# shaohua-pan/RobustCap

Hardware: AMD Instinct MI355X
Metric: body-frames/sec (sig_mp fwd + FK) at batch 256 (higher is better)
Workload: dtype f32; 1 GPU; synthetic 60 fps, 6 IMU + 33 keypoints, batch 256 x 1448 frames per GPU (256 bodies in total, weak scaling), confidence schedule 'mixed', seeded random weights (63.4 M params); batch_per_gpu=256, bodies_total=256, frames=1448, conf=mixed, parallelism=dp1 (sequence sharding)

## Files before the change

### include/robustcap_hip.h

```cpp
#ifndef ROBUSTCAP_HIP_H
#define ROBUSTCAP_HIP_H

#include <stdint.h>

#ifdef __cplusplus
extern "C" {
#endif

typedef struct rc_ctx rc_ctx;

typedef enum {
    RC_OK = 0,
    RC_ERR_INVALID = -1,
    RC_ERR_HIP = -2,
    RC_ERR_STATE = -3,
    RC_ERR_UNKNOWN_KEY = -4
} rc_status;

typedef struct {
    double conf_lo, conf_hi;
    float contact_threshold;
    float distance_threshold;
    float height_threshold;
    double tran_filter_num;
// ... 16 lines not shown
int rc_get_params(const rc_ctx* ctx, rc_params* out);
int rc_set_params(rc_ctx* ctx, const rc_params* p);

int rc_load_weight(rc_ctx* ctx, const char* key, const float* host, int64_t numel);
int rc_finalize_weights(rc_ctx* ctx);

int rc_set_body(rc_ctx* ctx, const int32_t* parent, const float* J, const float* w33, const float* v33);

int rc_set_gravity(rc_ctx* ctx, const float* gravity_host);

int rc_reset(rc_ctx* ctx, const uint8_t* row_mask, void* stream);

int rc_step(rc_ctx* ctx, const float* j2dc, const float* accc, const float* oric, const float* first_tran,
            uint32_t flags, float* pose_out, float* tran_out, void* stream);

int rc_sequence(rc_ctx* ctx, int32_t T, const float* j2dc, int64_t rs_j2d, const float* accc, int64_t rs_acc,
                const float* oric, int64_t rs_ori, const float* first_tran, uint32_t flags, float* pose_out,
                int64_t rs_pose, float* tran_out, int64_t rs_tran, void* stream);

int rc_sequence_rows(rc_ctx* ctx, int32_t T, const int32_t* len_host, const float* j2dc, int64_t rs_j2d, const float* accc,
                     int64_t rs_acc, const float* oric, int64_t rs_ori, const float* first_tran, uint32_t flags, float* pose_out,
                     int64_t rs_pose, float* tran_out, int64_t rs_tran, void* stream);
int rc_get_sequence_row_frames(rc_ctx* ctx, int64_t* body_frames);

int rc_set_gemm_mode(rc_ctx* ctx, int32_t mode);
int rc_get_gemm_mode(const rc_ctx* ctx);
int rc_default_gemm_mode(int32_t total_rows);
int rc_initial_gemm_mode(int32_t total_rows);

int rc_set_sequence_mode(rc_ctx* ctx, int32_t mode, int32_t min_frames);
int rc_get_sequence_stats(rc_ctx* ctx, int64_t* wave_frames, int64_t* stepped_frames, int64_t* ticks);
int rc_get_launch_stats(rc_ctx* ctx, int64_t* lds_launches, int64_t* other_wide_launches);
int rc_get_launch_stats_w32(rc_ctx* ctx, int64_t* w32_launches);
int rc_set_resident(rc_ctx* ctx, int32_t enable, int32_t workgroups);
int rc_get_resident_stats(rc_ctx* ctx, int64_t* segments, int64_t* aborts);
int rc_plan_sequence(const int8_t* codes, int32_t B, int32_t T, const int32_t* pend, uint32_t flags, int32_t use_vision_updater,
                     uint8_t* mode_out);
int rc_plan_wave(const int8_t* codes, int32_t B, int32_t T, int32_t t0, const int32_t* first_reach, const int32_t* pend,
                 int32_t use_imu_updater, int32_t use_vision_updater, int32_t* frame_at, int64_t frame_at_cap,
                 int32_t* n_ticks, int32_t* n_prep, int32_t* counts, double* est_us);
int rc_plan_wave_rows(const int8_t* codes, int32_t B, int32_t T, int32_t t0, const int32_t* len, const int32_t* first_reach,
                      const int32_t* pend, int32_t use_imu_updater, int32_t use_vision_updater, int32_t* frame_at, int64_t frame_at_cap,
                      int32_t* n_ticks, int32_t* n_prep, int32_t* counts, double* est_us);

int rc_live_begin(rc_ctx* ctx);
int rc_live_step(rc_ctx* ctx, const float* j2dc_host, const float* accc_host, const float* oric_host,
                 const float* first_tran_host, uint32_t flags, float* pose_host, float* tran_host);
int rc_live_end(rc_ctx* ctx);
int rc_get_live_stats(rc_ctx* ctx, int64_t* lean_frames, int64_t* full_frames);
int rc_get_live_prestep(rc_ctx* ctx, int64_t* presteps, int32_t* available);
int rc_get_live_replayed(rc_ctx* ctx, int64_t* frames);
int rc_get_live_spin(rc_ctx* ctx, int64_t* taken, int64_t* lost);
int rc_get_live_profile(rc_ctx* ctx, double* avg_us4);
int rc_get_live_last_profile(rc_ctx* ctx, double* us6);
int rc_get_live_backend(rc_ctx* ctx, int32_t* lean_captured, int32_t* aql, char* note, int32_t note_len);

int rc_r6d_to_rotmat(const float* r6d, float* R, int64_t n, void* stream);
int rc_axis_angle_to_rotmat(const float* aa, float* R, int64_t n, void* stream);
int rc_rotmat_to_axis_angle(const float* R, float* aa, int64_t n, void* stream);
int rc_rotmat_to_r6d(const float* R, float* r6d, int64_t n, void* stream);
int rc_angle_between(const float* R1, const float* R2, float* out, int64_t n, void* stream);
int rc_lerp(const float* a, const float* b, double t, float* out, int64_t n, void* stream);
int rc_normalize_rows(const float* x, float* out, float* norm, int64_t rows, int32_t width, void* stream);
int rc_bbox_normalise(const float* kp, float* out, int64_t n, void* stream);
int rc_conf_mean(const float* j2dc, int64_t n, double lo, double hi, float* mean, int8_t* code, void* stream);
int rc_shape_body(rc_ctx* ctx, const float* v_template, const float* shapedirs, const float* J_regressor, const float* beta,
// ... 142 lines not shown
```

### robustcap_amd/_lib.py

```python
import ctypes as C
import os

_HERE = os.path.dirname(os.path.abspath(__file__))
LIB_PATH = os.environ.get("RC_LIB_PATH") or os.path.join(_HERE, "csrc", "librobustcap_hip.so")
HEADER_PATH = os.path.join(os.path.dirname(_HERE), "include", "robustcap_hip.h")

RC_FLAG_FIRST_FRAME = 1


class RcParams(C.Structure):
    _fields_ = [("conf_lo", C.c_double), ("conf_hi", C.c_double),
                ("contact_threshold", C.c_float), ("distance_threshold", C.c_float),
                ("height_threshold", C.c_float), ("tran_filter_num", C.c_double),
                ("use_flat_floor", C.c_int32), ("use_vision_updater", C.c_int32),
                ("use_imu_updater", C.c_int32), ("live", C.c_int32),
                ("update_vision_freq", C.c_int32), ("use_reproj_opt", C.c_int32), ("smooth", C.c_float),
                ("reserved", C.c_int32)]


class RcSmplifyInfo(C.Structure):
    _fields_ = [("status", C.c_int32), ("n_iter", C.c_int32), ("n_eval", C.c_int32), ("reserved", C.c_int32),
                ("first_loss", C.c_double), ("final_loss", C.c_double), ("host_ms", C.c_double), ("device_ms", C.c_double)]


OBJECTIVE_FN = C.CFUNCTYPE(C.c_double, C.c_void_p, C.POINTER(C.c_double), C.POINTER(C.c_double), C.c_int64)


class RobustcapLibraryError(RuntimeError):
    pass


_P, _I32, _I64, _U32, _F = C.c_void_p, C.c_int32, C.c_int64, C.c_uint32, C.c_float
SIGNATURES = {
    "rc_create": (_I32, [_I32, _I32, C.POINTER(_P)]),
    "rc_destroy": (_I32, [_P]),
    "rc_last_error": (C.c_char_p, [_P]),
    "rc_default_params": (_I32, [_I32, C.POINTER(RcParams)]),
    "rc_get_params": (_I32, [_P, C.POINTER(RcParams)]),
    "rc_set_params": (_I32, [_P, C.POINTER(RcParams)]),
    "rc_load_weight": (_I32, [_P, C.c_char_p, _P, _I64]),
    "rc_finalize_weights": (_I32, [_P]),
    "rc_set_body": (_I32, [_P, _P, _P, _P, _P]),
    "rc_set_gravity": (_I32, [_P, _P]),
    "rc_reset": (_I32, [_P, _P, _P]),
    "rc_step": (_I32, [_P, _P, _P, _P, _P, _U32, _P, _P, _P]),
    "rc_sequence": (_I32, [_P, _I32, _P, _I64, _P, _I64, _P, _I64, _P, _U32, _P, _I64, _P, _I64, _P]),
    "rc_sequence_rows": (_I32, [_P, _I32, _P, _P, _I64, _P, _I64, _P, _I64, _P, _U32, _P, _I64, _P, _I64, _P]),
    "rc_get_sequence_row_frames": (_I32, [_P, C.POINTER(_I64)]),
    "rc_set_gemm_mode": (_I32, [_P, _I32]),
    "rc_get_gemm_mode": (_I32, [_P]),
    "rc_default_gemm_mode": (_I32, [_I32]),
    "rc_initial_gemm_mode": (_I32, [_I32]),
    "rc_set_sequence_mode": (_I32, [_P, _I32, _I32]),
    "rc_get_sequence_stats": (_I32, [_P, C.POINTER(_I64), C.POINTER(_I64), C.POINTER(_I64)]),
    "rc_get_launch_stats": (_I32, [_P, C.POINTER(_I64), C.POINTER(_I64)]),
    "rc_get_launch_stats_w32": (_I32, [_P, C.POINTER(_I64)]),
    "rc_set_resident": (_I32, [_P, _I32, _I32]),
    "rc_get_resident_stats": (_I32, [_P, C.POINTER(_I64), C.POINTER(_I64)]),
    "rc_plan_sequence": (_I32, [_P, _I32, _I32, _P, _U32, _I32, _P]),
    "rc_plan_wave": (_I32, [_P, _I32, _I32, _I32, _P, _P, _I32, _I32, _P, _I64, C.POINTER(_I32), C.POINTER(_I32), _P, _P]),
    "rc_plan_wave_rows": (_I32, [_P, _I32, _I32, _I32, _P, _P, _P, _I32, _I32, _P, _I64, C.POINTER(_I32), C.POINTER(_I32), _P, _P]),
    "rc_live_begin": (_I32, [_P]),
    "rc_live_step": (_I32, [_P, _P, _P, _P, _P, _U32, _P, _P]),
    "rc_live_end": (_I32, [_P]),
    "rc_get_live_stats": (_I32, [_P, _P, _P]),
    "rc_get_live_prestep": (_I32, [_P, _P, _P]),
    "rc_get_live_replayed": (_I32, [_P, _P]),
    "rc_get_live_spin": (_I32, [_P, _P, _P]),
    "rc_get_live_profile": (_I32, [_P, _P]),
    "rc_get_live_last_profile": (_I32, [_P, _P]),
    "rc_get_live_backend": (_I32, [_P, _P, _P, _P, _I32]),
    "rc_get_fusion_state": (_I32, [_P, _P, _P]),
    "rc_r6d_to_rotmat": (_I32, [_P, _P, _I64, _P]),
    "rc_axis_angle_to_rotmat": (_I32, [_P, _P, _I64, _P]),
    "rc_rotmat_to_axis_angle": (_I32, [_P, _P, _I64, _P]),
    "rc_rotmat_to_r6d": (_I32, [_P, _P, _I64, _P]),
    "rc_angle_between": (_I32, [_P, _P, _P, _I64, _P]),
    "rc_lerp": (_I32, [_P, _P, C.c_double, _P, _I64, _P]),
    "rc_normalize_rows": (_I32, [_P, _P, _P, _I64, _I32, _P]),
    "rc_bbox_normalise": (_I32, [_P, _P, _I64, _P]),
    "rc_conf_mean": (_I32, [_P, _I64, C.c_double, C.c_double, _P, _P, _P]),
    "rc_shape_body": (_I32, [_P, _P, _P, _P, _P, _I32, _P, _P]),
    "rc_fk_r": (_I32, [_P, _P, _P, _I64, _P]),
    "rc_bone_to_joint": (_I32, [_P, _P, _P, _I64, _P]),
    "rc_joint_to_bone": (_I32, [_P, _P, _P, _I64, _P]),
    "rc_zero_pose": (_I32, [_P, _P, _P, _P]),
    "rc_ik_r": (_I32, [_P, _P, _P, _I64, _P]),
    "rc_fk_bone": (_I32, [_P, _P, _P, _I64, _P]),
    "rc_body_fk": (_I32, [_P, _P, _P, _P, _P, _P, _I64, _P]),
# ... 101 lines not shown
```

### robustcap_amd/csrc/rc_api.cpp

```cpp
#include "../../include/robustcap_hip.h"
#include "rc_ctx.h"

#include <algorithm>
#include <cmath>
#include <cstdio>
#include <cstdlib>
#include <cstring>
#include <map>
#include <string>
#include <thread>
#include <vector>

static thread_local std::string g_create_error;

int fail(rc_ctx* ctx, int code, const std::string& msg) {
    if (ctx) ctx->err = msg; else g_create_error = msg;
    return code;
}

namespace {

const int kInit[3][2] = {{69, 512}, {512, 1024}, {1024, 2048}};

template <typename Body>
// ... 988 lines not shown
        if (ids[i] < 0 || ids[i] > 32) return fail(ctx, RC_ERR_INVALID, "rc_set_ignored_landmarks: id outside 0..32");
        m |= 1ull << ids[i];
    }
    ctx->ign_mask = m;
    return RC_OK;
}
int rc_reproj_residual(rc_ctx* ctx, const float* pose, const float* tran, const float* kp, const float* K, float sigma, float* loss,
                       int64_t T, void* stream) {
    if (!ctx || !ctx->have_body) return ctx ? fail(ctx, RC_ERR_STATE, "rc_reproj_residual: body not set") : RC_ERR_INVALID;
    if (T == 0) return RC_OK;
    if (T < 0 || !pose || !tran || !kp || !K || !loss) return fail(ctx, RC_ERR_INVALID, "rc_reproj_residual: null buffer");
    rc_launch_residual(ctx->body, pose, tran, kp, K, sigma, ctx->ign_mask, loss, T, (hipStream_t)stream);
    HIP_TRY(ctx, hipGetLastError());
    return RC_OK;
}

int rc_lstm_step(rc_ctx* ctx, const char* net, const float* x, const uint8_t* row_mask, float* y, void* stream) {
    if (!ctx || !net || !x || !y) return RC_ERR_INVALID;
    if (!ctx->have_weights) return fail(ctx, RC_ERR_STATE, "rc_lstm_step: weights not finalized");
    const int ni = net_index(net);
    if (ni < 0) return fail(ctx, RC_ERR_INVALID, std::string("rc_lstm_step: unknown net ") + net);
    hipStream_t st = (hipStream_t)stream;
    const NetDev& n = ctx->net[ni];
    if (int rc = flush_pending(ctx, st)) return rc;
    rc_launch_pack_rows(x, n.in, n.in, ctx->xtmp, 256, ctx->B, st);
    Stage s{ni, row_mask ? 255 : 0, ctx->xtmp, 256, Out{y, n.out, 0, false}};
    for (int phase = 0; phase < 4; ++phase) {
        GemmProblem p = phase == 0 ? lin1_problem(ctx, s) : (phase == 3 ? lin2_problem(ctx, s) : lstm_problem(ctx, s, phase - 1));
        if (int rc = launch_problems(ctx, {p}, row_mask, st)) return rc;
    }
    return mark_eager(ctx, st);
}

namespace {
bool camera_constants(const float* K, const float* Tcw, CamConst* cam, float* g_out) {
    for (int q = 0; q < 9; ++q) if (!std::isfinite(K[q])) return false;
    for (int q = 0; q < 12; ++q) if (!std::isfinite(Tcw[q])) return false;
    const double a = K[0], b = K[1], c = K[2], d = K[3], e = K[4], f = K[5], g = K[6], h = K[7], i = K[8];
    const double det = a * (e * i - f * h) - b * (d * i - f * g) + c * (d * h - e * g);
    if (det == 0.0) return false;
    const double inv[9] = {(e * i - f * h) / det, (c * h - b * i) / det, (b * f - c * e) / det,
                           (f * g - d * i) / det, (a * i - c * g) / det, (c * d - a * f) / det,
                           (d * h - e * g) / det, (b * g - a * h) / det, (a * e - b * d) / det};
    for (int q = 0; q < 9; ++q) if (!std::isfinite((float)inv[q])) return false;
    for (int q = 0; q < 9; ++q) cam->Kinv[q] = (float)inv[q];
    for (int r = 0; r < 3; ++r)
        for (int q = 0; q < 3; ++q) cam->R[3 * r + q] = Tcw[4 * r + q];
    for (int r = 0; r < 3; ++r) g_out[r] = -cam->R[3 * r + 1];
    return true;
}
}

int rc_camera_inputs(const float* kp, const float* acc, const float* ori, const float* K, const float* Tcw, float* j2dc,
                     float* accc, float* oric, float* g_out, int64_t n, void* stream) {
    if (!K || !Tcw || !g_out || n < 0) return RC_ERR_INVALID;
    if (n > 0 && (!kp || !acc || !ori || !j2dc || !accc || !oric)) return RC_ERR_INVALID;
    CamConst cam;
    if (!camera_constants(K, Tcw, &cam, g_out)) return RC_ERR_INVALID;
    if (n == 0) return RC_OK;
    rc_launch_camera_inputs(kp, acc, ori, cam, j2dc, accc, oric, n, (hipStream_t)stream);
    return hipGetLastError() == hipSuccess ? RC_OK : RC_ERR_HIP;
}

int rc_camera_inputs_rows(const float* kp_norm, const float* imu_acc_w, const float* imu_ori_w, const int32_t* seq_of_row,
                          const int32_t* len, const float* K_host, const float* Tcw_host, float image_w, float image_h,
                          int32_t n_rows, int32_t Tmax, float* j2dc, float* accc, float* oric, float* gravity_out_host,
// ... 66 lines not shown
```

### robustcap_amd/csrc/rc_ctx.h

```cpp
#pragma once
#include "../../include/robustcap_hip.h"
#include "rc_internal.h"

#include <map>
#include <string>
#include <type_traits>
#include <utility>
#include <vector>

struct NetSpec { const char* name; int in, H, out; };
const NetSpec kNets[6] = {{"rnn2", 72, 512, 69},  {"rnn3", 141, 512, 3},   {"rnn4", 171, 1280, 69},
                          {"rnn6", 240, 1024, 3}, {"rnn7", 141, 512, 144}, {"rnn8", 141, 512, 2}};
enum { N2 = 0, N3 = 1, N4 = 2, N6 = 3, N7 = 4, N8 = 5 };

inline int round_up(int x, int m) { return (x + m - 1) / m * m; }

struct Dense {
    float* W = nullptr; float* b = nullptr;
    void* Ws = nullptr;
    float* Wrm = nullptr;
    int K = 0, N = 0, Kp = 0, Np = 0;
    int mr = 2, nc = 4;
};
struct NetDev {
// ... 70 lines not shown
int tune_env(const char* name, int dflt);
int check_ready(rc_ctx* ctx);
rc_params_dev dev_params(const rc_params& p);
int step_impl(rc_ctx* ctx, const FrameIO& io, uint32_t flags, hipStream_t st, bool with_tr = true, bool skip_prep = false,
              const FrameIO* next_io = nullptr, int n_live = -1);
template <typename T>
int dev_alloc(rc_ctx* ctx, T** p, size_t count, bool zero = true) {
    DevBuf<char> q;
    HIP_TRY(ctx, rc_alloc(q, count * sizeof(T)));
    if (zero) HIP_TRY(ctx, hipMemset(q.get(), 0, count * sizeof(T)));
    *p = reinterpret_cast<T*>(q.get());
    if (!ctx->alloc_weights) ctx->alloc_bytes.emplace_back(q.get(), count * sizeof(T));
    (ctx->alloc_weights ? ctx->weight_allocs : ctx->allocs).push_back(std::move(q));
    return RC_OK;
}
int gemm_create(rc_ctx* ctx);
struct Out { float* p; int ld; int col0; bool packed; };
struct Stage {
    int net; int flag_bit; const float* x; int ldx; Out y;
    const unsigned char* flags = nullptr;
    const float* x_alt = nullptr;
    int sel_bit = 0;
    int out_bit = 0;
    int rows_hint = -1;
};
GemmSeg seg(const float* base, int ld, int K, int mode = RC_PAR_NONE, long long stride = 0);
GemmProblem dense_problem(const rc_ctx* ctx, const Dense& d, GemmSeg a, Out out, bool relu, int flag_bit, const unsigned char* flags, int* steps,
                          bool open_step);
GemmProblem lin1_problem(const rc_ctx* c, const Stage& s);
GemmProblem lstm_problem(const rc_ctx* c, const Stage& s, int layer);
GemmProblem lin2_problem(const rc_ctx* c, const Stage& s);
bool tile_env(const char* name, int* mr, int* nc);
void pick_tile(int H, int rows, int* mr, int* nc);
bool gemm_split(const rc_ctx* c);
int gemm_mode(const rc_ctx* c);
void gemm_planes2_released(rc_ctx* ctx);
int gemm_planes2_ensure(rc_ctx* ctx);
void gemm_planes2_refresh(rc_ctx* ctx, int net, hipStream_t st);
bool lds_context(const rc_ctx* c);
bool lds_problem(const rc_ctx* c, int rows);
struct LdsRegion { float* slab; int* tickets; size_t tiles; };
int lds_region(rc_ctx* ctx, size_t r, LdsRegion* out);
int build_lds_problems(rc_ctx* ctx, const std::vector<GemmProblem>& ps, const unsigned char* flags_override, float* slab, int* tickets,
                       LdsProblem* out, int max_p, int* items, size_t* tiles_out, bool resident_order = false);
int launch_problems(rc_ctx* ctx, std::vector<GemmProblem> ps, const unsigned char* flags_override, hipStream_t st, bool fp32 = false,
                    hipEvent_t stop = nullptr, bool* launched = nullptr);
enum LaunchKind { LAUNCH_SHARED, LAUNCH_WIDE, LAUNCH_SMALL, LAUNCH_RESIDENT };
int timed_launch_impl(rc_ctx* ctx, hipStream_t st, LaunchKind kind, void (*issue)(void*), void* arg);
template <class F> int timed_launch(rc_ctx* ctx, hipStream_t st, LaunchKind kind, F&& issue) {
    return timed_launch_impl(ctx, st, kind, [](void* f) { (*static_cast<std::remove_reference_t<F>*>(f))(); }, &issue);
}
bool resident_launch_fits_timing(const rc_ctx* c);
void count_resident_launch(rc_ctx* ctx);
struct LiveLaunchScope { rc_ctx* ctx; explicit LiveLaunchScope(rc_ctx* c); ~LiveLaunchScope(); };
struct TimingSuspended { rc_ctx* ctx; bool was; explicit TimingSuspended(rc_ctx* c); ~TimingSuspended(); };
void seq_create(rc_ctx* ctx);
int seq_prepare(rc_ctx* ctx);
void seq_weights_changed(rc_ctx* ctx);
bool seq_is_engine_stream(const rc_ctx* ctx, hipStream_t st);
void live_create(rc_ctx* ctx);
void live_forget_last_frame(rc_ctx* ctx, bool rows_reset = false);
int live_discard_ahead(rc_ctx* ctx);
int mark_eager(rc_ctx* ctx, hipStream_t st);
bool live_session_open(const rc_ctx* ctx);
#pragma GCC visibility pop
```

### robustcap_amd/csrc/rc_gemm.hip

```cpp
#include "rc_internal.h"
#include <hip/hip_ext.h>
#include <cstdlib>


#ifdef RC_TRACE_TILES
__device__ unsigned long long* g_trace_buf = nullptr;
__device__ unsigned long long g_trace_cap = 0;
extern "C" int rc_trace_tiles_set(unsigned long long* buf, unsigned long long cap_records) {
    if (hipMemcpyToSymbol(HIP_SYMBOL(g_trace_buf), &buf, sizeof(buf)) != hipSuccess) return -1;
    return hipMemcpyToSymbol(HIP_SYMBOL(g_trace_cap), &cap_records, sizeof(cap_records)) == hipSuccess ? 0 : -1;
}
#define TRACE_T(i) do { if (threadIdx.x == 0) trace_t[i] = wall_clock64(); } while (0)
#else
#define TRACE_T(i) do { } while (0)
#endif

#ifndef LDS_PAD
#define LDS_PAD 16
#endif
#define RC_LDS_HEAD 192

#include "rc_gates.h"
#include "rc_mma.h"
__device__ __forceinline__ float sigmoidf_(float x) { return rc_gate_sigmoid(x); }
// ... 280 lines not shown
            r[2] = __smid(); r[3] = (unsigned long long)n_tile | ((unsigned long long)m_tile << 32);
            r[4] = trace_t[0]; r[5] = trace_t[1]; r[6] = trace_t[2]; r[7] = wall_clock64();
        }
    }
#endif
  }
}

#ifndef RC_LDS_FLOATS
#define RC_LDS_FLOATS (RC_LDS_HEAD + RC_NW * 64 * (16 * 8 + LDS_PAD))
#endif

#ifndef RC_WPS
#define RC_WPS 1
#endif
__device__ __forceinline__ bool locate_tile(const GemmLaunch& L, int& pi, int& m_tile, int& n_tile) {
    pi = 0;
#pragma unroll
    for (int q = 1; q < RC_MAX_PROB; ++q)
        if (q < L.n && (int)blockIdx.x >= L.p[q].wg_base) pi = q;
    const GemmProblem& P = L.p[pi];
    const int local = blockIdx.x - P.wg_base;
    if ((P.n_tiles & 7) == 0) {
        const int xcd = local & 7, s = local >> 3;
        m_tile = s % P.m_tiles;
        n_tile = (s / P.m_tiles) * 8 + xcd;
    } else {
        m_tile = local % P.m_tiles;
        n_tile = local / P.m_tiles;
    }
    return n_tile < P.n_tiles;
}

template <bool SPLIT, int NP = 3>
__device__ __forceinline__ void wide_tiles(const GemmLaunch& L, float* s_mem) {
    int pi, m_tile, n_tile;
    if (!locate_tile(L, pi, m_tile, n_tile)) return;
    const GemmProblem& P = L.p[pi];
    switch (P.mr * 16 + P.nc) {
        case 8 * 16 + 4: gemm_tile<8, 4, 2, true, SPLIT, true, false, (RC_SPLIT_W32 != 0 && NP == 3), NP>(P, L.B, m_tile, n_tile, s_mem); break;
        case 4 * 16 + 8: gemm_tile<4, 8, 2, true, SPLIT, true, false, (RC_SPLIT_W32 != 0 && NP == 3), NP>(P, L.B, m_tile, n_tile, s_mem); break;
        case 4 * 16 + 5: gemm_tile<4, 5, 2, true, SPLIT, true, false, (RC_SPLIT_W32 != 0 && NP == 3), NP>(P, L.B, m_tile, n_tile, s_mem); break;
        case 4 * 16 + 4: gemm_tile<4, 4, 2, true, SPLIT, true, false, (RC_SPLIT_W32 != 0 && NP == 3), NP>(P, L.B, m_tile, n_tile, s_mem); break;
        case 2 * 16 + 10: gemm_tile<2, 10, 2, true, SPLIT, true, false, (RC_SPLIT_W32 != 0 && NP == 3), NP>(P, L.B, m_tile, n_tile, s_mem); break;
        case 2 * 16 + 8: gemm_tile<2, 8, 2, true, SPLIT, true, false, (RC_SPLIT_W32 != 0 && NP == 3), NP>(P, L.B, m_tile, n_tile, s_mem); break;
        case 1 * 16 + 2: gemm_tile<1, 2, 8, true, SPLIT, true, false, (RC_SPLIT_W32 != 0 && NP == 3), NP>(P, L.B, m_tile, n_tile, s_mem); break;
        case 1 * 16 + 1: gemm_tile<1, 1, 8, true, SPLIT, true, false, (RC_SPLIT_W32 != 0 && NP == 3), NP>(P, L.B, m_tile, n_tile, s_mem); break;
        default: gemm_tile<2, 4, 2, true, SPLIT, true, false, (RC_SPLIT_W32 != 0 && NP == 3), NP>(P, L.B, m_tile, n_tile, s_mem); break;
    }
}

__global__ __launch_bounds__(RC_NW * 64, RC_WPS) void rc_gemm_kernel(const GemmLaunch L) {
    __shared__ __attribute__((aligned(16))) float s_mem[RC_LDS_FLOATS];
    wide_tiles<false>(L, s_mem);
}
__global__ __launch_bounds__(RC_NW * 64, RC_WPS) void rc_gemm_split_kernel(const GemmLaunch L) {
    __shared__ __attribute__((aligned(16))) float s_mem[RC_LDS_FLOATS];
    wide_tiles<true>(L, s_mem);
}
__global__ __launch_bounds__(RC_NW * 64, RC_WPS) void rc_gemm_split2_kernel(const GemmLaunch L) {
    __shared__ __attribute__((aligned(16))) float s_mem[RC_LDS_FLOATS];
    wide_tiles<true, 2>(L, s_mem);
}

__global__ __launch_bounds__(RC_NW * 64, RC_WPS) void rc_gemm_split48_w32_kernel(const GemmLaunch L) {
    __shared__ __attribute__((aligned(16))) float s_mem[RC_LDS_FLOATS];
    int pi, m_tile, n_tile;
    if (!locate_tile(L, pi, m_tile, n_tile)) return;
    gemm_tile<4, 8, 2, true, true, true, false, true>(L.p[pi], L.B, m_tile, n_tile, s_mem);
}

#define RC_MID_LDS_FLOATS (RC_LDS_HEAD + RC_NW * 32 * (16 * 4 + LDS_PAD))
template <bool SPLIT, int NP = 3>
__device__ __forceinline__ void mid_tiles(const GemmLaunch& L, float* s_mem) {
    int pi, m_tile, n_tile;
    if (!locate_tile(L, pi, m_tile, n_tile)) return;
    const GemmProblem& P = L.p[pi];
    switch (P.mr * 16 + P.nc) {
// ... 41 lines not shown
__global__ __launch_bounds__(RC_NW * 64, 4) void rc_gemm_small_split_kernel(const GemmLaunch L) {
    __shared__ __attribute__((aligned(16))) float s_mem[RC_SMALL_LDS_FLOATS];
    small_tiles<true>(L, s_mem);
}
__global__ __launch_bounds__(RC_NW * 64, 4) void rc_gemm_small_split2_kernel(const GemmLaunch L) {
    __shared__ __attribute__((aligned(16))) float s_mem[RC_SMALL_LDS_FLOATS];
    small_tiles<true, false, 2>(L, s_mem);
}

__global__ __launch_bounds__(256) void rc_planes2_kernel(const f32x4* __restrict__ W, u32x4* __restrict__ Ws2, long long n) {
    const long long t = (long long)blockIdx.x * 256 + threadIdx.x;
    if (t >= n) return;
    const long long blk = t >> 6;
    const int lane = (int)(t & 63);
    u32x4 h, m;
    split2_rn(W[(2 * blk) * 64 + lane], W[(2 * blk + 1) * 64 + lane], h, m);
    Ws2[(2 * blk) * 64 + lane] = h;
    Ws2[(2 * blk + 1) * 64 + lane] = m;
}
void rc_launch_planes2(const float* W, void* Ws2, int Np, int Kp, hipStream_t s) {
    const long long n = (long long)(Np / 16) * (Kp / 32) * 64;
    hipLaunchKernelGGL(rc_planes2_kernel, dim3((unsigned)((n + 255) / 256)), dim3(256), 0, s, reinterpret_cast<const f32x4*>(W),
                       reinterpret_cast<u32x4*>(Ws2), n);
}

bool rc_gemm_is_small(const GemmLaunch& L) {
    bool small = true;
    for (int q = 0; q < L.n; ++q) small = small && L.p[q].mr == 1 && L.p[q].nc <= 2;
    return small;
}

bool rc_gemm_is_mid(const GemmLaunch& L) {
    bool mid = true;
    for (int q = 0; q < L.n; ++q) mid = mid && L.p[q].mr <= 2 && L.p[q].nc <= 4 && !(L.p[q].mr == 2 && L.p[q].nc < 4);
    return mid;
}

bool rc_gemm_is_w32(const GemmLaunch& L) {
    if (rc_gemm_is_small(L) || rc_gemm_is_mid(L)) return false;
    bool one_reader = L.split == 1;
    for (int q = 0; q < L.n; ++q) one_reader = one_reader && L.p[q].mr == 4 && L.p[q].nc == 8 && L.p[q].m_tiles == 1;
    static const bool w32 = !std::getenv("RC_GEMM_W32") || std::atoi(std::getenv("RC_GEMM_W32")) != 0;
    return one_reader && w32;
}

void rc_launch_gemm(const GemmLaunch& L, int total_wg, hipStream_t s, hipEvent_t stop) {
    const dim3 g(total_wg), b(RC_NW * 64);
#define RC_GO(K) do { if (stop) hipExtLaunchKernelGGL(K, g, b, 0, s, nullptr, stop, 0, L); else hipLaunchKernelGGL(K, g, b, 0, s, L); } while (0)
    if (rc_gemm_is_small(L)) {
        bool single_reader = L.live != 0;
        for (int q = 0; q < L.n; ++q) single_reader = single_reader && L.p[q].m_tiles == 1;
        if (L.split == 2) RC_GO(rc_gemm_small_split2_kernel);
        else if (L.split) RC_GO(rc_gemm_small_split_kernel);
        else if (single_reader) RC_GO(rc_gemm_small_nt_kernel);
        else RC_GO(rc_gemm_small_kernel);
    } else if (rc_gemm_is_mid(L)) {
        if (L.split == 2) RC_GO(rc_gemm_mid_split2_kernel);
        else if (L.split) RC_GO(rc_gemm_mid_split_kernel);
        else RC_GO(rc_gemm_mid_kernel);
    } else {
        if (rc_gemm_is_w32(L)) RC_GO(rc_gemm_split48_w32_kernel);
        else if (L.split == 2) RC_GO(rc_gemm_split2_kernel);
        else if (L.split) RC_GO(rc_gemm_split_kernel);
        else RC_GO(rc_gemm_kernel);
    }
#undef RC_GO
}
// ... 1 lines not shown
```

### robustcap_amd/csrc/rc_gemm_api.cpp

```cpp
#include "../../include/robustcap_hip.h"
#include "rc_ctx.h"

#include <algorithm>
#include <cstdio>
#include <cstdlib>
#include <cstring>
#include <map>
#include <string>
#include <vector>

#define RC_SPLIT_MIN_BATCH 48
#define RC_TILE64_MIN_BATCH 192

#ifndef RC_NC1280
#define RC_NC1280 10
#endif

const int kLdsRegions = 12;

#pragma GCC visibility push(hidden)

struct GemmLauncher {
    int mode = 0;
    std::map<const void*, void*> planes2;
    bool live_launch = false;
    unsigned live_nt_mask = 63u;
    int tile4[2] = {4, 5}, tile6[2] = {4, 8}, tile378[2] = {4, 4}, tile2[2] = {0, 0};
    int trace_next = 0;
    bool timing = false;
    int timing_mode = 1;
    std::vector<std::pair<HipEvent, HipEvent>> ev_pool;
    size_t ev_used = 0;
    double timed_ms = 0.0;
    double timed_busy_ms = 0.0;
    long long timed_launches = 0;
    long long stat_wide_launches = 0;
    long long stat_lds_launches = 0;
    long long stat_w32_launches = 0;
    int lds_min_rows = 64;
    int lds_min_batch = 65;
    int lds_ksplit[3] = {1, 2, 2};
    bool lds_block_pick = true;
    DevBuf<float> lds_slab;
    DevBuf<int> lds_tickets;
    size_t lds_region_tiles = 0;
    unsigned lds_rot = 0;
};

void rc_gemm_free(GemmLauncher* g) { delete g; }

static int default_gemm_mode(int rows) { return tune_env("RC_GEMM_SPLIT", rows >= RC_SPLIT_MIN_BATCH ? 1 : 0) != 0 ? 1 : 0; }

static int initial_gemm_mode(int rows) { return tune_env("RC_GEMM_SPLIT", -1) == 2 ? 2 : default_gemm_mode(rows); }

int gemm_create(rc_ctx* ctx) {
    ctx->gemm.reset(new GemmLauncher());
    GemmLauncher& g = *ctx->gemm;
    const int batch = ctx->B;
    g.mode = initial_gemm_mode(batch);
    g.live_nt_mask = (unsigned)tune_env("RC_LIVE_NT_MASK", 63);
    g.lds_min_rows = tune_env("RC_LDS_MIN_ROWS", std::min(160, std::max(64, batch / 2)));
    g.lds_min_batch = tune_env("RC_LDS_MIN_BATCH", g.lds_min_batch);
    g.lds_block_pick = tune_env("RC_LDS_BLOCK_PICK", 1) != 0;
    g.lds_ksplit[0] = tune_env("RC_LDS_KSPLIT_512", 1) == 1 ? 1 : 2;
    g.lds_ksplit[1] = tune_env("RC_LDS_KSPLIT_1024", batch <= 160 ? 1 : 2) == 1 ? 1 : 2;
    g.lds_ksplit[2] = tune_env("RC_LDS_KSPLIT_1280", 2) == 1 ? 1 : 2;
    const struct { const char* knob; int* tile; int H; } tiles[4] = {{"RC_TILE_RNN6", g.tile6, 1024}, {"RC_TILE_S2H512", g.tile378, 512},
                                                                     {"RC_TILE_RNN2", g.tile2, 512}, {"RC_TILE_RNN4", g.tile4, 1280}};
    for (const auto& t : tiles) tile_env(t.knob, &t.tile[0], &t.tile[1]);
    for (const auto& t : tiles)
        if (t.tile[1] > 0 && t.H % (4 * t.tile[1]) != 0)
            return fail(nullptr, RC_ERR_INVALID, std::string("rc_create: ") + t.knob + " tile width of " + std::to_string(4 * t.tile[1]) +
                                                 " units does not divide H = " + std::to_string(t.H));
    return RC_OK;
}

bool gemm_split(const rc_ctx* c) { return c->gemm->mode != 0; }
int gemm_mode(const rc_ctx* c) { return c->gemm->mode; }
bool lds_context(const rc_ctx* c) { return c->gemm->mode != 0 && c->gemm->lds_min_rows > 0 && c->B >= c->gemm->lds_min_batch; }
bool lds_problem(const rc_ctx* c, int rows) { return lds_context(c) && rows >= c->gemm->lds_min_rows; }

LiveLaunchScope::LiveLaunchScope(rc_ctx* c) : ctx(c) { ctx->gemm->live_launch = true; }
LiveLaunchScope::~LiveLaunchScope() { ctx->gemm->live_launch = false; }
TimingSuspended::TimingSuspended(rc_ctx* c) : ctx(c), was(c->gemm->timing) { ctx->gemm->timing = false; }
TimingSuspended::~TimingSuspended() { ctx->gemm->timing = was; }

GemmSeg seg(const float* base, int ld, int K, int mode, long long stride) {
    GemmSeg s{};
    s.base = base; s.ld = ld; s.K = K; s.par_mode = mode; s.par_stride = stride;
    return s;
}

GemmProblem dense_problem(const rc_ctx* ctx, const Dense& d, GemmSeg a, Out out, bool relu, int flag_bit,
                          const unsigned char* flags, int* steps, bool open_step) {
    GemmProblem p{};
    a.K = d.Kp;
    p.seg[0] = a;
    p.seg[1] = seg(a.base, a.ld, 0);
    p.W = d.W; p.Ws = d.Ws; p.bias = d.b; p.out = out.p; p.ldo = out.ld; p.N = d.N; p.out_col0 = out.col0; p.out_packed = out.packed ? 1 : 0;
    p.steps = steps; p.flags = flags; p.flag_bit = flag_bit;
    p.epi = relu ? RC_EPI_RELU : RC_EPI_DENSE;
    p.open_step = open_step ? 1 : 0;
    const bool narrow = ctx->B <= 16 || d.N <= 160;
    const int mr = narrow ? 1 : d.mr, nc = narrow ? 1 : d.nc;
    p.n_tiles = nc == 1 ? (d.N + 15) / 16 : d.Np / (16 * nc);
    p.m_tiles = (ctx->B + 16 * mr - 1) / (16 * mr); p.Kp = d.Kp; p.nc = nc; p.mr = mr;
    return p;
}

bool tile_env(const char* name, int* mr, int* nc) {
    const char* v = std::getenv(name);
    int a = 0, b = 0;
    if (!v || std::sscanf(v, "%dx%d", &a, &b) != 2) return false;
    const int code = a * 16 + b;
    for (int ok : {2 * 16 + 4, 4 * 16 + 4, 8 * 16 + 4, 2 * 16 + 8, 4 * 16 + 8, 2 * 16 + 10, 4 * 16 + 5})
        if (code == ok) { *mr = a; *nc = b; return true; }
    return false;
}

void pick_tile(int H, int rows, int* mr, int* nc) {
    if (rows >= 128) { *mr = 2; *nc = H == 1280 ? RC_NC1280 : (H == 1024 ? 8 : 4); return; }
    if (rows > 16) { *mr = 2; *nc = rows >= 64 ? 4 : 2; if (*nc == 2) { *mr = 1; } return; }
    *mr = 1; *nc = 1;
}

GemmProblem lin1_problem(const rc_ctx* c, const Stage& s) {
    const NetDev& n = c->net[s.net];
    GemmProblem p = dense_problem(c, n.lin1, seg(s.x, s.ldx, 0), Out{n.x1, n.H, 0, true}, true, s.flag_bit,
                                  s.flags ? s.flags : c->fb.flags, n.steps, true);
    if (s.rows_hint >= 0 && s.rows_hint <= 16) {
        p.mr = 1; p.nc = 1; p.n_tiles = (n.lin1.N + 15) / 16;
    }
    if (s.rows_hint >= 0 && s.rows_hint < c->B) p.m_tiles = (s.rows_hint + 16 * p.mr - 1) / (16 * p.mr);
    p.alt_base = s.x_alt; p.sel_flags = c->fb.flags; p.sel_bit = s.x_alt ? s.sel_bit : 0;
    p.nt = (c->gemm->live_nt_mask >> s.net) & 1u;
    return p;
}
GemmProblem lstm_problem(const rc_ctx* c, const Stage& s, int layer) {
    const GemmLauncher& g = *c->gemm;
    const NetDev& n = c->net[s.net];
    const long long BH = (long long)c->Bp * n.H;
    GemmProblem p{};
    if (layer == 0) p.seg[0] = seg(n.x1, n.H, n.H);
    else p.seg[0] = seg(n.h, n.H, n.H, RC_PAR_DST, BH);
    p.seg[1] = seg(n.h + layer * RC_HBUF * BH, n.H, n.H, RC_PAR_SRC, BH);
    p.W = n.Wl[layer]; p.Ws = n.Wls[layer]; p.bias = n.bl[layer];
    p.hstate = n.h + layer * RC_HBUF * BH; p.cstate = n.c + layer * (long long)c->B * n.H; p.h_par_stride = BH; p.H = n.H;
    p.steps = n.steps; p.flags = s.flags ? s.flags : c->fb.flags; p.flag_bit = s.flag_bit;
    p.epi = RC_EPI_LSTM;
    int mr, nc;
    pick_tile(n.H, s.rows_hint < 0 ? c->B : s.rows_hint, &mr, &nc);
    if (s.rows_hint < 0 && c->B >= RC_TILE64_MIN_BATCH) {
        if (s.net == N6 && g.tile6[0]) { mr = g.tile6[0]; nc = g.tile6[1]; }
        if ((s.net == N3 || s.net == N7 || s.net == N8) && g.tile378[0]) { mr = g.tile378[0]; nc = g.tile378[1]; }
        if (s.net == N2 && g.tile2[0]) { mr = g.tile2[0]; nc = g.tile2[1]; }
        if (s.net == N4 && g.tile4[0]) { mr = g.tile4[0]; nc = g.tile4[1]; }
// ... 271 lines not shown
            ++written;
            if (r != g) ++bad;
        }
        std::fprintf(stderr, "[dbg dense] N %d Kp %d alt %d: %zu of %zu written elements differ\n", ps[i].N, ps[i].Kp, ps[i].alt_base ? 1 : 0, bad, written);
    }
    return RC_OK;
}

int launch_problems(rc_ctx* ctx, std::vector<GemmProblem> ps, const unsigned char* flags_override, hipStream_t st, bool fp32, hipEvent_t stop,
                    bool* launched) {
    GemmLauncher& g = *ctx->gemm;
    if (launched) *launched = false;
    if (ps.empty()) return RC_OK;
    if (dense_items_selftest_wanted(ctx, ps, st, fp32)) return dense_items_selftest(ctx, ps, flags_override, st);
    {
        std::vector<GemmProblem> lds, rest;
        for (GemmProblem& p : ps) {
            if (p.mr == 16) {
                if (g.mode != 0 && !fp32 && p.epi == RC_EPI_LSTM && (int)lds.size() < RC_LDS_MAXP) { lds.push_back(p); continue; }
                p.mr = 4; p.nc = 8; p.m_tiles *= 4;
            }
            rest.push_back(p);
        }
        if (!lds.empty()) {
            if (!rest.empty()) if (int rc = launch_problems(ctx, rest, flags_override, st, fp32)) return rc;
            return launch_lds(ctx, lds, flags_override, st, stop, launched);
        }
    }
    if ((int)ps.size() > RC_MAX_PROB) {
        std::vector<GemmProblem> head(ps.begin(), ps.begin() + RC_MAX_PROB), tail(ps.begin() + RC_MAX_PROB, ps.end());
        if (int rc = launch_problems(ctx, head, flags_override, st, fp32)) return rc;
        return launch_problems(ctx, tail, flags_override, st, fp32, stop, launched);
    }
    GemmLaunch L{};
    const int base = lay_out_launch(ctx, ps, flags_override, fp32 ? 0 : g.mode, L);
    if (base == -2) return fail(ctx, RC_ERR_STATE, "gemm mode 2: a matrix has no weight planes");
    if (base < 0) return fail(ctx, RC_ERR_INVALID, "too many fused problems");
    g.trace_next = (g.trace_next + base) & 0x3fffffff;
    const bool small = rc_gemm_is_small(L);
    if (!small) g.stat_wide_launches += 1;
    if (rc_gemm_is_w32(L)) g.stat_w32_launches += 1;
    if (int rc = timed_launch(ctx, st, small ? LAUNCH_SMALL : LAUNCH_WIDE, [&] { rc_launch_gemm(L, base, st, stop); })) return rc;
    if (launched && stop) *launched = true;
    HIP_TRY(ctx, hipGetLastError());
    return RC_OK;
}

#pragma GCC visibility pop

int rc_ctx_gemm_split(rc_ctx* ctx) { return ctx->gemm->mode != 0 ? 1 : 0; }
int rc_ctx_gemm_mode(rc_ctx* ctx) { return ctx->gemm->mode; }

extern "C" {

int rc_set_gemm_mode(rc_ctx* ctx, int32_t mode) {
    if (!ctx || mode < 0 || mode > 2)
        return ctx ? fail(ctx, RC_ERR_INVALID, "rc_set_gemm_mode: 0 (fp32 MFMA), 1 (split-bf16, six products) or 2 (two rounded bf16 terms, three products)") : RC_ERR_INVALID;
    if (mode == ctx->gemm->mode) return RC_OK;
    rc_live_end(ctx);
    const int was = ctx->gemm->mode;
    ctx->gemm->mode = mode;
    if (int rc = gemm_planes2_ensure(ctx)) { ctx->gemm->mode = was; return rc; }
    return RC_OK;
}
int rc_get_gemm_mode(const rc_ctx* ctx) { return ctx ? ctx->gemm->mode : RC_ERR_INVALID; }
int rc_default_gemm_mode(int32_t total_rows) { return default_gemm_mode(total_rows); }
int rc_initial_gemm_mode(int32_t total_rows) { return initial_gemm_mode(total_rows); }

int rc_get_launch_stats_w32(rc_ctx* ctx, int64_t* w32_launches) {
    if (!ctx || !w32_launches) return RC_ERR_INVALID;
    *w32_launches = ctx->gemm->stat_w32_launches;
    return RC_OK;
}

int rc_get_launch_stats(rc_ctx* ctx, int64_t* tick_launches, int64_t* other_wide_launches) {
    if (!ctx) return RC_ERR_INVALID;
    if (tick_launches) *tick_launches = ctx->gemm->stat_lds_launches;
    if (other_wide_launches) *other_wide_launches = ctx->gemm->stat_wide_launches;
    return RC_OK;
}

int rc_gemm_timing(rc_ctx* ctx, int32_t enable) {
    if (!ctx) return RC_ERR_INVALID;
    GemmLauncher& g = *ctx->gemm;
    g.timing = enable != 0;
    if (enable) g.timing_mode = enable == 2 ? 2 : (enable == 3 ? 3 : 1);
    if (enable) { g.ev_used = 0; g.timed_ms = 0.0; g.timed_launches = 0; g.timed_busy_ms = 0.0; }
    return RC_OK;
}
int rc_gemm_timing_read(rc_ctx* ctx, double* total_ms, int64_t* launches) {
    if (!ctx || !total_ms || !launches) return RC_ERR_INVALID;
    GemmLauncher& g = *ctx->gemm;
    std::vector<std::pair<double, double>> iv;
    iv.reserve(g.ev_used);
    for (size_t i = 0; i < g.ev_used; ++i) {
        HIP_TRY(ctx, hipEventSynchronize(g.ev_pool[i].second.get()));
        float ms = 0.f, t0 = 0.f;
        HIP_TRY(ctx, hipEventElapsedTime(&ms, g.ev_pool[i].first.get(), g.ev_pool[i].second.get()));
        if (i > 0) HIP_TRY(ctx, hipEventElapsedTime(&t0, g.ev_pool[0].first.get(), g.ev_pool[i].first.get()));
        iv.emplace_back((double)t0, (double)t0 + ms);
        g.timed_ms += ms;
        g.timed_launches += 1;
    }
    std::sort(iv.begin(), iv.end());
    double lo = 0.0, hi = -1.0;
    for (const auto& x : iv) {
        if (hi < lo || x.first > hi) { if (hi > lo) g.timed_busy_ms += hi - lo; lo = x.first; hi = x.second; }
        else if (x.second > hi) hi = x.second;
    }
    if (hi > lo) g.timed_busy_ms += hi - lo;
    g.ev_used = 0;
// ... 12 lines not shown
```

### robustcap_amd/csrc/rc_sequence_api.cpp

```cpp
#include "../../include/robustcap_hip.h"
#include "rc_ctx.h"

#include <algorithm>
#include <chrono>
#include <cstdio>
#include <cstring>
#include <initializer_list>
#include <vector>

#define RC_SPLIT_MAIN_MIN_BATCH 48

namespace {

enum { SEQ_STEPPED_TR = 0, SEQ_STEPPED = 1 };
const int kRing = 16;

enum { G_BIG = 0, G_REST = 1, G_LIN2 = 2 };
struct TickStage { int kind; int net; int stage; int group; };
const TickStage kTick[RC_TICK_PROB] = {
    {1, N4, 2, G_BIG}, {2, N4, 3, G_BIG}, {1, N6, 6, G_BIG}, {2, N6, 7, G_BIG},
    {1, N2, 2, G_REST}, {2, N2, 3, G_REST}, {1, N3, 6, G_REST}, {2, N3, 7, G_REST}, {1, N7, 6, G_REST}, {2, N7, 7, G_REST}, {1, N8, 6, G_REST}, {2, N8, 7, G_REST},
    {0, N4, 1, G_REST}, {0, N2, 1, G_REST}, {0, N6, 5, G_REST}, {0, N3, 5, G_REST}, {0, N7, 5, G_REST}, {0, N8, 5, G_REST},
    {3, N4, 4, G_LIN2}, {3, N2, 4, G_LIN2}, {3, N6, 8, G_LIN2}, {3, N3, 8, G_LIN2}, {3, N7, 8, G_LIN2}, {3, N8, 8, G_LIN2}};
const int kFuseStage = 4, kTailStage = 8, kInitStage = 5;
// ... 306 lines not shown
    static const int tile64_rows = tune_env("RC_SEQ_TILE64_ROWS", 33);
    static const bool rows_as_padded = tune_env("RC_SEQ_ROWS_AS_PADDED", 1) != 0;
    const int B = ctx->B;
    std::vector<GemmProblem> ps;
    for (int qi = 0; qi < W2_PROB; ++qi) {
        const int q = qi < 4 ? (qi ^ 2) : qi;
        if (w2_group(q, eng == ENG_TRI) != g) continue;
        const int e = k - w2_stage(q);
        if (e < 0 || e >= P.n_prep) continue;
        const int net = q < RC_TICK_PROB ? kTick[q].net : -1;
        const int kind = q < RC_TICK_PROB ? kTick[q].kind : 4;
        const int riders = P.n_rider[e];
        const int rows = kind == 4 ? P.n_reach[e] : ((net == N4 || net == N6) ? P.n_vis[e] + riders : P.n_valid[e]);
        if (rows <= 0) continue;
        const int rows_k = kind == 4 ? rows : rows + (rows_as_padded ? P.done(e) : 0);
        GemmProblem p = ctx->seq->wave2_prob[(size_t)(e % kRing) * W2_PROB + q];
        if (kind == 0 || kind == 1) {
            float* x1 = e % 3 == 0 ? ctx->net[net].x1 : (e % 3 == 1 ? ctx->seq->x1_alt[net] : ctx->seq->x1_alt2[net]);
            if (kind == 0) p.out = x1; else p.seg[0].base = x1;
        }
        if (kind == 1 || kind == 2) {
            const NetDev& n = ctx->net[net];
            int mr, nc;
            if (lds_problem(ctx, rows_k)) {
                mr = 16; nc = 8;
            } else if (gemm_split(ctx) && rows_k >= tile64_rows) {
                const int* t = n.H == 512 ? tiles.t5 : (n.H == 1024 ? tiles.t6 : tiles.t4);
                mr = t[0]; nc = t[1];
            } else {
                pick_tile(n.H, rows_k, &mr, &nc);
            }
            p.mr = mr; p.nc = nc; p.n_tiles = n.H / (4 * nc);
        } else if (kind == 0 || kind == 4) {
            if (rows_k <= 16) { p.mr = 1; p.nc = 1; p.n_tiles = (p.N + 15) / 16; }
            else if (kind == 0 && gemm_split(ctx) && rows_k >= tile64_rows) {
                const int np = round_up(p.N, 64);
                if (np % 128 == 0) { p.mr = 4; p.nc = 8; p.n_tiles = np / 128; }
            }
        }
        p.m_tiles = (rows + 16 * p.mr - 1) / (16 * p.mr);
        if (rows == B && kind != 4) {
            p.flags = nullptr; p.flag_bit = 0;
            if (riders == 0 && (net == N4 || net == N6) && P.n_vis[e] == B) {
                p.alt_base = nullptr; p.sel_flags = nullptr; p.sel_bit = 0; p.out_flags = nullptr; p.out_bit = 0;
            }
        }
        ps.push_back(p);
    }
    if (g != G_LIN2) {
        int total = 0;
        for (const GemmProblem& p : ps) total += p.n_tiles * p.m_tiles;
        if (total > 0 && total <= 128)
            for (GemmProblem& p : ps)
                if (p.epi == RC_EPI_LSTM && p.mr == 4 && p.nc == 8) { p.nc = 4; p.n_tiles *= 2; }
    }
    return ps;
}

struct WaveSeg {
    rc_ctx* ctx; const WavePlan& P; const FrameIO& io0; hipStream_t st, aux;
    WaveEngine eng; WaveTiles tiles; rc_params_dev prm; WavePrep wp; WaveTail wt;
    int rows(const std::vector<int>& v, int tick) const { return tick >= 0 && tick < P.n_prep ? v[tick] : 0; }
    std::vector<GemmProblem> group(int k, int g) const { return collect(ctx, P, eng, tiles, k, g); }
};

void wave_prep(WaveSeg& S, int k) {
    if (k >= S.P.n_prep) return;
    S.wp.frame_at = S.ctx->seq->frame_at_d.get() + (size_t)k * S.ctx->B;
    S.wp.first_tick = k == 0 ? 1 : 0;
    rc_launch_prep_wave(S.ctx->seq->ring2[k % kRing], S.io0, S.prm, S.ctx->B, S.wp, S.aux);
}
// ... 474 lines not shown
```

Before: 1.288 million body-frames/s.

## Widen few-row dense tiles in wide launches and read launch params from kernarg

```diff
diff --git a/include/robustcap_hip.h b/include/robustcap_hip.h
--- a/include/robustcap_hip.h
+++ b/include/robustcap_hip.h
@@ -72,6 +72,11 @@
 int rc_get_sequence_stats(rc_ctx* ctx, int64_t* wave_frames, int64_t* stepped_frames, int64_t* ticks);
 int rc_get_launch_stats(rc_ctx* ctx, int64_t* lds_launches, int64_t* other_wide_launches);
 int rc_get_launch_stats_w32(rc_ctx* ctx, int64_t* w32_launches);
+int rc_chain_tile_query(int32_t kind, int32_t N, int32_t rows_k, int32_t batch, int32_t gemm_mode, int32_t wide_launch, int32_t few_row_nc,
+                        int32_t* mr, int32_t* nc, int32_t* n_tiles);
+int rc_chain_lin1_workgroups(int32_t batch, int32_t n_valid, int32_t n_vis, int32_t n_reach, int32_t few_row_nc, int32_t* workgroups);
+int rc_dense_probe(rc_ctx* ctx, int32_t kind, int32_t N, int32_t K, const float* W_host, const float* b_host, int32_t rows_k, const float* x,
+                   const uint8_t* row_mask, float* y, int32_t* mr, int32_t* nc, void* stream);
 int rc_set_resident(rc_ctx* ctx, int32_t enable, int32_t workgroups);
 int rc_get_resident_stats(rc_ctx* ctx, int64_t* segments, int64_t* aborts);
 int rc_plan_sequence(const int8_t* codes, int32_t B, int32_t T, const int32_t* pend, uint32_t flags, int32_t use_vision_updater,
diff --git a/robustcap_amd/_lib.py b/robustcap_amd/_lib.py
--- a/robustcap_amd/_lib.py
+++ b/robustcap_amd/_lib.py
@@ -55,6 +55,9 @@
     "rc_get_sequence_stats": (_I32, [_P, C.POINTER(_I64), C.POINTER(_I64), C.POINTER(_I64)]),
     "rc_get_launch_stats": (_I32, [_P, C.POINTER(_I64), C.POINTER(_I64)]),
     "rc_get_launch_stats_w32": (_I32, [_P, C.POINTER(_I64)]),
+    "rc_chain_tile_query": (_I32, [_I32] * 7 + [C.POINTER(_I32)] * 3),
+    "rc_chain_lin1_workgroups": (_I32, [_I32] * 5 + [C.POINTER(_I32)]),
+    "rc_dense_probe": (_I32, [_P, _I32, _I32, _I32, _P, _P, _I32, _P, _P, _P, C.POINTER(_I32), C.POINTER(_I32), _P]),
     "rc_set_resident": (_I32, [_P, _I32, _I32]),
     "rc_get_resident_stats": (_I32, [_P, C.POINTER(_I64), C.POINTER(_I64)]),
     "rc_plan_sequence": (_I32, [_P, _I32, _I32, _P, _U32, _I32, _P]),
diff --git a/robustcap_amd/csrc/rc_api.cpp b/robustcap_amd/csrc/rc_api.cpp
--- a/robustcap_amd/csrc/rc_api.cpp
+++ b/robustcap_amd/csrc/rc_api.cpp
@@ -1044,6 +1044,22 @@
     return mark_eager(ctx, st);
 }
 
+int rc_dense_probe(rc_ctx* ctx, int32_t kind, int32_t N, int32_t K, const float* W_host, const float* b_host, int32_t rows_k, const float* x,
+                   const uint8_t* row_mask, float* y, int32_t* mr, int32_t* nc, void* stream) {
+    if (!ctx || !W_host || !b_host || !x || !y || !mr || !nc) return RC_ERR_INVALID;
+    if ((kind != 0 && kind != 4) || N < 16 || K < 1 || N > 4096 || K > 4096 || N % 16 != 0)
+        return fail(ctx, RC_ERR_INVALID, "rc_dense_probe: kind 0 or 4, N a multiple of 16 within 16 .. 4096, K within 1 .. 4096");
+    hipStream_t st = (hipStream_t)stream;
+    Dense d;
+    if (int rc = make_dense(ctx, d, std::vector<float>(W_host, W_host + (size_t)N * K), std::vector<float>(b_host, b_host + N), N, K)) return rc;
+    float* xpk = nullptr;
+    if (int rc = dev_alloc(ctx, &xpk, (size_t)ctx->Bp * d.Kp)) return rc;
+    rc_launch_pack_rows(x, K, K, xpk, d.Kp, ctx->B, st);
+    if (int rc = gemm_probe_dense(ctx, d, kind, rows_k > 0 ? rows_k : ctx->B, xpk, row_mask, y, mr, nc, st)) return rc;
+    HIP_TRY(ctx, hipStreamSynchronize(st));
+    return RC_OK;
+}
+
 namespace {
 bool camera_constants(const float* K, const float* Tcw, CamConst* cam, float* g_out) {
     for (int q = 0; q < 9; ++q) if (!std::isfinite(K[q])) return false;
diff --git a/robustcap_amd/csrc/rc_ctx.h b/robustcap_amd/csrc/rc_ctx.h
--- a/robustcap_amd/csrc/rc_ctx.h
+++ b/robustcap_amd/csrc/rc_ctx.h
@@ -126,6 +126,10 @@
 GemmProblem lin2_problem(const rc_ctx* c, const Stage& s);
 bool tile_env(const char* name, int* mr, int* nc);
 void pick_tile(int H, int rows, int* mr, int* nc);
+struct TileShape { int mr, nc, n_tiles; };
+TileShape tick_dense_shape(int kind, int N, int rows_k, int batch, bool split, int tile64_rows);
+int gemm_probe_dense(rc_ctx* ctx, const Dense& d, int kind, int rows_k, const float* xpk, const unsigned char* row_mask, float* y, int* mr, int* nc,
+                     hipStream_t st);
 bool gemm_split(const rc_ctx* c);
 int gemm_mode(const rc_ctx* c);
 void gemm_planes2_released(rc_ctx* ctx);
diff --git a/robustcap_amd/csrc/rc_gemm.hip b/robustcap_amd/csrc/rc_gemm.hip
--- a/robustcap_amd/csrc/rc_gemm.hip
+++ b/robustcap_amd/csrc/rc_gemm.hip
@@ -336,8 +336,17 @@
     return n_tile < P.n_tiles;
 }
 
+__device__ __forceinline__ const GemmLaunch& launch_in_kernarg(const GemmLaunch& L) {
+#if defined(__HIP_DEVICE_COMPILE__)
+    return *(const GemmLaunch*)__builtin_amdgcn_kernarg_segment_ptr();
+#else
+    return L;
+#endif
+}
+
 template <bool SPLIT, int NP = 3>
-__device__ __forceinline__ void wide_tiles(const GemmLaunch& L, float* s_mem) {
+__device__ __forceinline__ void wide_tiles(const GemmLaunch& L_, float* s_mem) {
+    const GemmLaunch& L = launch_in_kernarg(L_);
     int pi, m_tile, n_tile;
     if (!locate_tile(L, pi, m_tile, n_tile)) return;
     const GemmProblem& P = L.p[pi];
@@ -348,6 +357,8 @@
         case 4 * 16 + 4: gemm_tile<4, 4, 2, true, SPLIT, true, false, (RC_SPLIT_W32 != 0 && NP == 3), NP>(P, L.B, m_tile, n_tile, s_mem); break;
         case 2 * 16 + 10: gemm_tile<2, 10, 2, true, SPLIT, true, false, (RC_SPLIT_W32 != 0 && NP == 3), NP>(P, L.B, m_tile, n_tile, s_mem); break;
         case 2 * 16 + 8: gemm_tile<2, 8, 2, true, SPLIT, true, false, (RC_SPLIT_W32 != 0 && NP == 3), NP>(P, L.B, m_tile, n_tile, s_mem); break;
+        case 1 * 16 + 8: gemm_tile<1, 8, 4, true, SPLIT, true, false, (RC_SPLIT_W32 != 0 && NP == 3), NP>(P, L.B, m_tile, n_tile, s_mem); break;
+        case 1 * 16 + 4: gemm_tile<1, 4, 8, true, SPLIT, true, false, (RC_SPLIT_W32 != 0 && NP == 3), NP>(P, L.B, m_tile, n_tile, s_mem); break;
         case 1 * 16 + 2: gemm_tile<1, 2, 8, true, SPLIT, true, false, (RC_SPLIT_W32 != 0 && NP == 3), NP>(P, L.B, m_tile, n_tile, s_mem); break;
         case 1 * 16 + 1: gemm_tile<1, 1, 8, true, SPLIT, true, false, (RC_SPLIT_W32 != 0 && NP == 3), NP>(P, L.B, m_tile, n_tile, s_mem); break;
         default: gemm_tile<2, 4, 2, true, SPLIT, true, false, (RC_SPLIT_W32 != 0 && NP == 3), NP>(P, L.B, m_tile, n_tile, s_mem); break;
@@ -455,7 +466,8 @@
 
 bool rc_gemm_is_mid(const GemmLaunch& L) {
     bool mid = true;
-    for (int q = 0; q < L.n; ++q) mid = mid && L.p[q].mr <= 2 && L.p[q].nc <= 4 && !(L.p[q].mr == 2 && L.p[q].nc < 4);
+    for (int q = 0; q < L.n; ++q)
+        mid = mid && L.p[q].mr <= 2 && L.p[q].nc <= 4 && !(L.p[q].mr == 2 && L.p[q].nc < 4) && !(L.p[q].mr == 1 && L.p[q].nc > 2);
     return mid;
 }
 
diff --git a/robustcap_amd/csrc/rc_gemm_api.cpp b/robustcap_amd/csrc/rc_gemm_api.cpp
--- a/robustcap_amd/csrc/rc_gemm_api.cpp
+++ b/robustcap_amd/csrc/rc_gemm_api.cpp
@@ -16,6 +16,7 @@
 #define RC_NC1280 10
 #endif
 
+const int kFewRowNcDefault = 8;
 const int kLdsRegions = 12;
 
 #pragma GCC visibility push(hidden)
@@ -41,6 +42,8 @@
     int lds_min_batch = 65;
     int lds_ksplit[3] = {1, 2, 2};
     bool lds_block_pick = true;
+    int few_row_nc = kFewRowNcDefault;
+    bool few_row_force = false;
     DevBuf<float> lds_slab;
     DevBuf<int> lds_tickets;
     size_t lds_region_tiles = 0;
@@ -65,6 +68,8 @@
     g.lds_ksplit[0] = tune_env("RC_LDS_KSPLIT_512", 1) == 1 ? 1 : 2;
     g.lds_ksplit[1] = tune_env("RC_LDS_KSPLIT_1024", batch <= 160 ? 1 : 2) == 1 ? 1 : 2;
     g.lds_ksplit[2] = tune_env("RC_LDS_KSPLIT_1280", 2) == 1 ? 1 : 2;
+    const int few_nc = tune_env("RC_CHAIN_FEW_ROW_NC", g.few_row_nc);
+    g.few_row_nc = (few_nc == 4 || few_nc == 8) ? few_nc : 0;
     const struct { const char* knob; int* tile; int H; } tiles[4] = {{"RC_TILE_RNN6", g.tile6, 1024}, {"RC_TILE_S2H512", g.tile378, 512},
                                                                      {"RC_TILE_RNN2", g.tile2, 512}, {"RC_TILE_RNN4", g.tile4, 1280}};
     for (const auto& t : tiles) tile_env(t.knob, &t.tile[0], &t.tile[1]);
@@ -122,6 +127,32 @@
     if (rows >= 128) { *mr = 2; *nc = H == 1280 ? RC_NC1280 : (H == 1024 ? 8 : 4); return; }
     if (rows > 16) { *mr = 2; *nc = rows >= 64 ? 4 : 2; if (*nc == 2) { *mr = 1; } return; }
     *mr = 1; *nc = 1;
+}
+
+const int kTile64RowsDefault = 33;
+
+TileShape tick_dense_shape(int kind, int N, int rows_k, int batch, bool split, int tile64_rows) {
+    if (rows_k <= 16 || batch <= 16 || N <= 160) return TileShape{1, 1, (N + 15) / 16};
+    if (kind == 0 && split && rows_k >= tile64_rows && round_up(N, 64) % 128 == 0) return TileShape{4, 8, round_up(N, 64) / 128};
+    return TileShape{2, 4, round_up(N, 64) / 64};
+}
+static bool wide_shape(int mr, int nc) { return !(mr == 1 && nc <= 2) && !(mr == 2 && nc == 4); }
+static int few_row_nc(int knob, bool dense, int mr, int nc, int N) {
+    if (!knob || !dense || mr != 1 || nc != 1) return 0;
+    if (N % (16 * knob) == 0) return knob;
+    return (knob == 8 && N % 64 == 0) ? 4 : 0;
+}
+static void few_row_tiles(int knob, std::vector<GemmProblem>& ps, bool force) {
+    bool wide = force;
+    for (const GemmProblem& p : ps) wide = wide || wide_shape(p.mr, p.nc);
+    if (!wide) return;
+    for (GemmProblem& p : ps)
+        if (const int nc = few_row_nc(knob, p.epi != RC_EPI_LSTM, p.mr, p.nc, p.N)) { p.nc = nc; p.n_tiles = p.N / (16 * nc); }
+}
+static int launch_workgroups(const std::vector<GemmProblem>& ps) {
+    int wg = 0;
+    for (const GemmProblem& p : ps) wg += round_up(p.n_tiles * p.m_tiles, 8);
+    return wg;
 }
 
 GemmProblem lin1_problem(const rc_ctx* c, const Stage& s) {
@@ -459,6 +490,7 @@
         if (int rc = launch_problems(ctx, head, flags_override, st, fp32)) return rc;
         return launch_problems(ctx, tail, flags_override, st, fp32, stop, launched);
     }
+    if (!g.live_launch) few_row_tiles(g.few_row_nc, ps, g.few_row_force);
     GemmLaunch L{};
     const int base = lay_out_launch(ctx, ps, flags_override, fp32 ? 0 : g.mode, L);
     if (base == -2) return fail(ctx, RC_ERR_STATE, "gemm mode 2: a matrix has no weight planes");
@@ -473,6 +505,28 @@
     return RC_OK;
 }
 
+int gemm_probe_dense(rc_ctx* ctx, const Dense& d, int kind, int rows_k, const float* xpk, const unsigned char* row_mask, float* y, int* mr, int* nc,
+                     hipStream_t st) {
+    GemmLauncher& g = *ctx->gemm;
+    GemmProblem p = dense_problem(ctx, d, seg(xpk, d.Kp, 0), Out{y, d.N, 0, kind == 0}, kind == 0, row_mask ? 255 : 0, row_mask, nullptr, false);
+    const TileShape t = tick_dense_shape(kind, d.N, rows_k, ctx->B, g.mode != 0, kTile64RowsDefault);
+    p.mr = t.mr; p.nc = t.nc; p.n_tiles = t.n_tiles;
+    p.m_tiles = (ctx->B + 16 * p.mr - 1) / (16 * p.mr);
+    if (g.mode == 2 && !g.planes2.count(d.Ws)) {
+        uint16_t* q = nullptr;
+        if (int rc = dev_alloc(ctx, &q, (size_t)d.Np * d.Kp * 2, false)) return rc;
+        rc_launch_planes2(d.W, q, d.Np, d.Kp, st);
+        g.planes2[d.Ws] = q;
+    }
+    std::vector<GemmProblem> shaped{p};
+    few_row_tiles(g.few_row_nc, shaped, true);
+    *mr = shaped[0].mr; *nc = shaped[0].nc;
+    g.few_row_force = true;
+    const int rc = launch_problems(ctx, {p}, row_mask, st, g.mode == 0);
+    g.few_row_force = false;
+    return rc;
+}
+
 #pragma GCC visibility pop
 
 int rc_ctx_gemm_split(rc_ctx* ctx) { return ctx->gemm->mode != 0 ? 1 : 0; }
@@ -504,6 +558,33 @@
     if (!ctx) return RC_ERR_INVALID;
     if (tick_launches) *tick_launches = ctx->gemm->stat_lds_launches;
     if (other_wide_launches) *other_wide_launches = ctx->gemm->stat_wide_launches;
+    return RC_OK;
+}
+
+int rc_chain_tile_query(int32_t kind, int32_t N, int32_t rows_k, int32_t batch, int32_t gemm_mode, int32_t wide_launch, int32_t few_row_nc_knob,
+                        int32_t* mr, int32_t* nc, int32_t* n_tiles) {
+    if (!mr || !nc || !n_tiles || N < 1 || rows_k < 1 || batch < 1 || (kind != 0 && kind != 4)) return RC_ERR_INVALID;
+    TileShape t = tick_dense_shape(kind, N, rows_k, batch, gemm_mode != 0, kTile64RowsDefault);
+    if (wide_launch)
+        if (const int w = few_row_nc(few_row_nc_knob < 0 ? kFewRowNcDefault : few_row_nc_knob, true, t.mr, t.nc, N)) { t.nc = w; t.n_tiles = N / (16 * w); }
+    *mr = t.mr; *nc = t.nc; *n_tiles = t.n_tiles;
+    return RC_OK;
+}
+
+int rc_chain_lin1_workgroups(int32_t batch, int32_t n_valid, int32_t n_vis, int32_t n_reach, int32_t few_row_nc_knob, int32_t* workgroups) {
+    if (!workgroups || batch < 1 || n_valid < 0 || n_vis < 0 || n_reach < 0 || n_valid > batch || n_vis > n_valid || n_reach > n_valid) return RC_ERR_INVALID;
+    std::vector<GemmProblem> ps;
+    auto add = [&](int kind, int N, int rows) {
+        if (rows <= 0) return;
+        const TileShape t = tick_dense_shape(kind, N, rows, batch, true, kTile64RowsDefault);
+        GemmProblem p{};
+        p.epi = RC_EPI_RELU; p.N = N; p.mr = t.mr; p.nc = t.nc; p.n_tiles = t.n_tiles; p.m_tiles = (rows + 16 * t.mr - 1) / (16 * t.mr);
+        ps.push_back(p);
+    };
+    for (int i = 0; i < 6; ++i) add(0, kNets[i].H, (i == N4 || i == N6) ? n_vis : n_valid);
+    for (int N : {512, 1024, 2048}) add(4, N, n_reach);
+    few_row_tiles(few_row_nc_knob < 0 ? kFewRowNcDefault : few_row_nc_knob, ps, false);
+    *workgroups = launch_workgroups(ps);
     return RC_OK;
 }
 
diff --git a/robustcap_amd/csrc/rc_sequence_api.cpp b/robustcap_amd/csrc/rc_sequence_api.cpp
--- a/robustcap_amd/csrc/rc_sequence_api.cpp
+++ b/robustcap_amd/csrc/rc_sequence_api.cpp
@@ -362,11 +362,8 @@
             }
             p.mr = mr; p.nc = nc; p.n_tiles = n.H / (4 * nc);
         } else if (kind == 0 || kind == 4) {
-            if (rows_k <= 16) { p.mr = 1; p.nc = 1; p.n_tiles = (p.N + 15) / 16; }
-            else if (kind == 0 && gemm_split(ctx) && rows_k >= tile64_rows) {
-                const int np = round_up(p.N, 64);
-                if (np % 128 == 0) { p.mr = 4; p.nc = 8; p.n_tiles = np / 128; }
-            }
+            const TileShape t = tick_dense_shape(kind, p.N, rows_k, B, gemm_split(ctx), tile64_rows);
+            p.mr = t.mr; p.nc = t.nc; p.n_tiles = t.n_tiles;
         }
         p.m_tiles = (rows + 16 * p.mr - 1) / (16 * p.mr);
         if (rows == B && kind != 4) {
```

Result: no change. 1.292 million body-frames/s, median of 6 (+0.3%).
